# awentzonline/tartangan

Measured on AMD Instinct MI355X. Metric: images/sec (G+D step), higher is better.
Workload: dtype f32; 1 GPU; 128:3 SA-GAN cnn G+D step (R1 penalty, Adam x2, EMA), 128x128 RGB, batch 64/GPU, global batch 64; trainer=cnn, gan_config=128:3, global_batch=64, parallelism=dp1, hip_graphs=True

## Files before the change

tartangan_amd/csrc/conv.hip:

```cpp
#include <cstdlib>
#include <type_traits>
#include <utility>

#include "common.h"

namespace {

typedef float f32x16 __attribute__((ext_vector_type(16)));
typedef float f32x4 __attribute__((ext_vector_type(4)));

constexpr int CT_THREADS = 256;

template <int TH_, int TW_, int NI_>
struct Geo {
  static constexpr int TH = TH_, TW = TW_, NI = NI_, NPIX = TH_ * TW_ * NI_;
  static_assert(NPIX == 512 || NPIX == 256 || NPIX == 64, "a pixel tile is 512 / 256 pixels (waves split pixels) or 64 (waves split K)");
  static constexpr int PPW = (NPIX == 64) ? 64 : NPIX / 4;
  static_assert(TW_ % 4 == 0, "rows are staged as float4");
};
using G4 = Geo<4, 4, 16>;
using G8 = Geo<8, 8, 4>;
using G16 = Geo<16, 16, 1>;
using GX = Geo<8, 32, 1>;
using G4k = Geo<4, 4, 4>;
// ... 692 lines not shown
#pragma unroll
        for (int m = 0; m < MT; ++m)
          a[m] = DGRAD ? wl[lane_a + (g * KG) * F::RS + m * MF * 9 - tap] : wl[lane_a + m * MF * F::RS + (g * KG) * 9 + tap];
#pragma unroll
        for (int n = 0; n < NT; ++n) b[n] = pl[lane_b[n] + (g * KG) * P::CIS + kh * P::PWS + kw];
#pragma unroll
        for (int m = 0; m < MT; ++m)
#pragma unroll
          for (int n = 0; n < NT; ++n) {
            if constexpr (MF == 32)
              acc[m][n] = __builtin_amdgcn_mfma_f32_32x32x2f32(a[m], b[n], acc[m][n], 0, 0, 0);
            else
              acc[m][n] = __builtin_amdgcn_mfma_f32_16x16x4f32(a[m], b[n], acc[m][n], 0, 0, 0);
          }
      }
    }
    if (prio) __builtin_amdgcn_s_setprio(3);
    if (DB) buf ^= 1;
  }
#ifdef TG_DIAG_STAMPS
  {
    const uint64_t st_c1 = __builtin_amdgcn_s_memtime(), st_r1 = __builtin_amdgcn_s_memrealtime();
    const int slot = blockIdx.y * gridDim.x + blockIdx.x;
    if (threadIdx.x == 0 && slot < TG_DIAG_SLOTS) { tg_diag_stamps[2 * slot] = st_c1 - st_c0; tg_diag_stamps[2 * slot + 1] = st_r1 - st_r0; }
    st_mfma += st_c1 - st_last;
    if (lane == 0 && slot < TG_DIAG_SLOTS) {
      unsigned long long* ph = tg_diag_phases + (slot * 4 + wave) * 4;
      ph[0] = st_wait; ph[1] = st_bar; ph[2] = st_issue; ph[3] = st_mfma;
    }
  }
#endif
  if constexpr (WK) {
    __syncthreads();
    float* red = lds;
#pragma unroll
    for (int m = 0; m < MT; ++m)
#pragma unroll
      for (int n = 0; n < NT; ++n)
#pragma unroll
        for (int r = 0; r < NREG; ++r) red[(((wave * MT + m) * NT + n) * NREG + r) * 64 + lane] = acc[m][n][r];
    __syncthreads();
    constexpr int PW_ = MT * NT * NREG * 64;
#pragma unroll
    for (int m = 0; m < MT; ++m)
#pragma unroll
      for (int n = 0; n < NT; ++n)
#pragma unroll
        for (int r = 0; r < NREG; ++r) {
          const int e = ((m * NT + n) * NREG + r) * 64 + lane;
          acc[m][n][r] = (red[e] + red[PW_ + e]) + (red[2 * PW_ + e] + red[3 * PW_ + e]);
        }
  }
#ifdef TG_DIAG_STAMPS
  if ((xcd_swizzle & 2) && acc[0][0][0] != 12345.678f) return;
#endif
  Core::epilogue(acc, bias, residual, y, s, tc, co0, pix0, j, h, wave);
#ifdef TG_DIAG_STAMPS
  {
    const uint64_t e0 = __builtin_amdgcn_s_memtime();
    asm volatile("s_waitcnt vmcnt(0)" ::: "memory");
    const uint64_t e1 = __builtin_amdgcn_s_memtime();
    const int slot = blockIdx.y * gridDim.x + blockIdx.x;
    if (lane == 0 && slot < TG_DIAG_SLOTS) {
      unsigned long long* ph = tg_diag_life + (slot * 4 + wave) * 4;
      ph[0] = st_c0 - st_begin; ph[1] = e0 - st_c0; ph[2] = e1 - e0; ph[3] = st_setup - st_begin;
    }
  }
#endif
}

template <int CO, int PX>
__global__ void __launch_bounds__(256)
conv1x1_direct_kernel(const float* __restrict__ x, const float* __restrict__ w, const float* __restrict__ bias,
                      const float* __restrict__ residual, float* __restrict__ y, int Cin, int Cout, int HW, int w_so, int w_si) {
  __shared__ __attribute__((aligned(16))) float wl[1024];
  for (int e = threadIdx.x; e < Cin * CO; e += 256) {
    const int ci = e / CO, co = e - ci * CO;
    wl[e] = co < Cout ? w[co * w_so + ci * w_si] : 0.f;
  }
  __syncthreads();
  const int b = blockIdx.y;
  const int p = (blockIdx.x * 256 + threadIdx.x) * PX;
  if (p >= HW) return;
  const float* xb = x + (int64_t)b * Cin * HW + p;
  float acc[CO][PX];
#pragma unroll
  for (int co = 0; co < CO; ++co)
#pragma unroll
    for (int u = 0; u < PX; ++u) acc[co][u] = 0.f;
#pragma unroll 4
  for (int ci = 0; ci < Cin; ++ci) {
    float xv[PX];
    if (PX == 4) {
      const float4 t = *reinterpret_cast<const float4*>(xb + (int64_t)ci * HW);
      xv[0] = t.x; xv[1] = t.y; xv[2] = t.z; xv[3] = t.w;
    } else {
      xv[0] = xb[(int64_t)ci * HW];
    }
#pragma unroll
    for (int c4 = 0; c4 < CO / 4; ++c4) {
      const float4 wv = *reinterpret_cast<const float4*>(&wl[ci * CO + 4 * c4]);
      const float ww[4] = {wv.x, wv.y, wv.z, wv.w};
#pragma unroll
      for (int k = 0; k < 4; ++k)
#pragma unroll
        for (int u = 0; u < PX; ++u) acc[4 * c4 + k][u] = fmaf(ww[k], xv[u], acc[4 * c4 + k][u]);
    }
  }
  const int64_t ob = (int64_t)b * Cout * HW + p;
#pragma unroll
  for (int co = 0; co < CO; ++co) {
    if (co >= Cout) break;
    const float bv = bias ? bias[co] : 0.f;
    float o[PX];
#pragma unroll
    for (int u = 0; u < PX; ++u) o[u] = acc[co][u] + bv;
    const int64_t off = ob + (int64_t)co * HW;
    if (PX == 4) {
      if (residual) {
        const float4 r = *reinterpret_cast<const float4*>(residual + off);
        o[0] += r.x; o[1] += r.y; o[2] += r.z; o[3] += r.w;
      }
      *reinterpret_cast<float4*>(y + off) = make_float4(o[0], o[1], o[2], o[3]);
    } else {
      if (residual) o[0] += residual[off];
      y[off] = o[0];
    }
  }
}

template <int CO>
static int launch_conv1x1_direct(const float* x, const float* w, const float* bias, const float* residual, float* y, Shape s,
                                 bool dgrad, hipStream_t st) {
  const int HW = s.H * s.W;
  const int w_so = dgrad ? 1 : s.Cin, w_si = dgrad ? s.Cout : 1;
  const bool vec = (HW % 4 == 0) && tg_aligned16(x) && tg_aligned16(y) && (!residual || tg_aligned16(residual));
  if (vec) {
    dim3 grid((HW / 4 + 255) / 256, s.B);
    conv1x1_direct_kernel<CO, 4><<<grid, 256, 0, st>>>(x, w, bias, residual, y, s.Cin, s.Cout, HW, w_so, w_si);
  } else {
    dim3 grid((HW + 255) / 256, s.B);
    conv1x1_direct_kernel<CO, 1><<<grid, 256, 0, st>>>(x, w, bias, residual, y, s.Cin, s.Cout, HW, w_so, w_si);
  }
  return tg_launch_status();
}
static inline int conv1x1_co(int Cout) { return Cout <= 4 ? 4 : 8; }
static inline bool conv1x1_direct_ok(const Shape& s) { return s.Cout <= 8 && s.Cin * conv1x1_co(s.Cout) <= 1024 && s.B <= 65535; }
static int launch_conv1x1(const float* x, const float* w, const float* bias, const float* residual, float* y, Shape s, bool dgrad,
                          hipStream_t st) {
  if (s.Cout <= 4) return launch_conv1x1_direct<4>(x, w, bias, residual, y, s, dgrad, st);
  return launch_conv1x1_direct<8>(x, w, bias, residual, y, s, dgrad, st);
}

struct ChanSegs {
  float* p[3];
  int start[4];
  __device__ __forceinline__ int find(int c) const { return c >= start[2] ? 2 : (c >= start[1] ? 1 : 0); }
  __device__ __forceinline__ int width(int k) const { return start[k + 1] - start[k]; }
};
static inline ChanSegs one_seg(const float* p, int channels) {
  ChanSegs g;
  g.p[0] = g.p[1] = g.p[2] = const_cast<float*>(p);
  g.start[0] = 0; g.start[1] = g.start[2] = g.start[3] = channels;
  return g;
}
static inline ChanSegs three_segs(const float* p0, const float* p1, const float* p2, int c0, int c1, int c2) {
  ChanSegs g;
  g.p[0] = const_cast<float*>(p0); g.p[1] = const_cast<float*>(p1); g.p[2] = const_cast<float*>(p2);
  g.start[0] = 0; g.start[1] = c0; g.start[2] = c0 + c1; g.start[3] = c0 + c1 + c2;
  return g;
}

template <int NCO>
__global__ void __launch_bounds__(256)
conv1x1_mfma_kernel(ChanSegs xs, const float* __restrict__ w, const float* __restrict__ bias,
                    const float* __restrict__ residual, ChanSegs ys, int Cin, int Cout, int HW, int64_t quads,
                    int w_so, int w_si) {
  const int lane = threadIdx.x & 63, j = lane & 15, h = lane >> 4;
  const int64_t q = ((int64_t)blockIdx.x * 4 + (threadIdx.x >> 6)) * 16 + j;
  const bool live = q < quads;
  const int qpp = HW >> 2;
  const int64_t b = live ? q / qpp : 0;
  const int p = live ? (int)(q - b * qpp) * 4 : 0;
  f32x4 acc[NCO][4];
#pragma unroll
  for (int m = 0; m < NCO; ++m)
#pragma unroll
    for (int r = 0; r < 4; ++r) acc[m][r] = f32x4{0.f, 0.f, 0.f, 0.f};
  int wrow[NCO];
#pragma unroll
  for (int m = 0; m < NCO; ++m) wrow[m] = min(16 * m + j, Cout - 1) * w_so;
  constexpr int U = 4;
  for (int k0 = 0; k0 < Cin; k0 += 4 * U) {
    float4 xv[U];
    float a[U][NCO];
#pragma unroll
    for (int u = 0; u < U; ++u) {
      const int ci = k0 + 4 * u + h;
      const bool ok = live && ci < Cin;
      const int cc = min(ci, Cin - 1);
      const int k = xs.find(cc);
      const float* src = xs.p[k] + ((b * xs.width(k) + (cc - xs.start[k])) * HW + p);
      xv[u] = ok ? *reinterpret_cast<const float4*>(src) : make_float4(0.f, 0.f, 0.f, 0.f);
#pragma unroll
      for (int m = 0; m < NCO; ++m) a[u][m] = (ci < Cin) ? w[wrow[m] + cc * w_si] : 0.f;
    }
#pragma unroll
    for (int u = 0; u < U; ++u) {
      const float bx[4] = {xv[u].x, xv[u].y, xv[u].z, xv[u].w};
#pragma unroll
      for (int m = 0; m < NCO; ++m)
#pragma unroll
        for (int r = 0; r < 4; ++r) acc[m][r] = __builtin_amdgcn_mfma_f32_16x16x4f32(a[u][m], bx[r], acc[m][r], 0, 0, 0);
    }
  }
  if (!live) return;
  const float* rb = residual ? residual + (b * Cout) * HW + p : nullptr;
#pragma unroll
  for (int m = 0; m < NCO; ++m)
#pragma unroll
    for (int i = 0; i < 4; ++i) {
      const int co = 16 * m + 4 * h + i;
      if (co >= Cout) continue;
      const float bv = bias ? bias[co] : 0.f;
      float4 o = make_float4(acc[m][0][i] + bv, acc[m][1][i] + bv, acc[m][2][i] + bv, acc[m][3][i] + bv);
      if (rb) {
        const float4 t = *reinterpret_cast<const float4*>(rb + (int64_t)co * HW);
        o.x += t.x; o.y += t.y; o.z += t.z; o.w += t.w;
      }
      const int k = ys.find(co);
      *reinterpret_cast<float4*>(ys.p[k] + ((b * ys.width(k) + (co - ys.start[k])) * HW + p)) = o;
    }
}

static inline bool conv1x1_mfma_ok(const float* x, const float* residual, const float* y, const Shape& s) {
  return (s.H * s.W) % 4 == 0 && s.Cout <= 128 && tg_aligned16(x) && tg_aligned16(y) && (!residual || tg_aligned16(residual));
}
static int launch_conv1x1_segs(ChanSegs xs, const float* w, const float* bias, const float* residual, ChanSegs ys, Shape s, bool dgrad,
                               hipStream_t st) {
  const int HW = s.H * s.W;
  const int64_t quads = (int64_t)s.B * (HW / 4);
  const int w_so = dgrad ? 1 : s.Cin, w_si = dgrad ? s.Cout : 1;
  const unsigned grid = (unsigned)((quads + 63) / 64);
  const int nco = (s.Cout + 15) / 16;
#define TG_1X1(N) conv1x1_mfma_kernel<N><<<grid, 256, 0, st>>>(xs, w, bias, residual, ys, s.Cin, s.Cout, HW, quads, w_so, w_si)
  if (nco <= 1) TG_1X1(1);
  else if (nco == 2) TG_1X1(2);
  else if (nco <= 4) TG_1X1(4);
  else TG_1X1(8);
#undef TG_1X1
  return tg_launch_status();
}
static int launch_conv1x1_mfma(const float* x, const float* w, const float* bias, const float* residual, float* y, Shape s, bool dgrad,
                               hipStream_t st) {
  return launch_conv1x1_segs(one_seg(x, s.Cin), w, bias, residual, one_seg(y, s.Cout), s, dgrad, st);
}

template <int KS> struct WgCfg {
  static constexpr int CKW = (KS == 3) ? 16 : 32;
  static constexpr int KK = KS * KS;
  static constexpr int NCOL = CKW * KK;
  static constexpr int NT = (NCOL + 15) / 16;
};
constexpr int WG_GYS = 256 + 4;

template <class G, int CT>
struct GyStager {
  static constexpr int Q = G::TW / 4;
  static constexpr int ROWS_PER_CO = G::NI * G::TH;
  static constexpr int ROWS = CT * ROWS_PER_CO;
  static constexpr int NV = (ROWS * Q + CT_THREADS - 1) / CT_THREADS;
  float4 v[NV];

  __device__ __forceinline__ void load(const float* __restrict__ gy, const Shape& s, int co0, const TileCoord& tc, bool vec) {
#pragma unroll
    for (int i = 0; i < NV; ++i) {
      const int e = threadIdx.x + i * CT_THREADS;
      float4 val = make_float4(0.f, 0.f, 0.f, 0.f);
      if (e < ROWS * Q) {
        const int q = e % Q, row = e / Q;
        const int r = row % G::TH;
        const int t = row / G::TH;
        const int img = t % G::NI, co = t / G::NI;
        const int b = tc.b0 + img, hh = tc.h0 + r, ww = tc.w0 + 4 * q;
        if (b < s.B && co0 + co < s.Cout && hh < s.H && ww < s.W) {
          const float* base = gy + ((((int64_t)tc.b0 * s.Cout + co0) * s.H + tc.h0) * s.W + tc.w0);
          const float* src = base + (__umul24(__umul24(img, s.Cout) + co, s.H * s.W) + __umul24(r, s.W) + 4 * q);
          if (vec) {
            val = *reinterpret_cast<const float4*>(src);
          } else {
            val.x = src[0];
            if (ww + 1 < s.W) val.y = src[1];
            if (ww + 2 < s.W) val.z = src[2];
            if (ww + 3 < s.W) val.w = src[3];
          }
        }
      }
      v[i] = val;
    }
  }

  __device__ __forceinline__ void store(float* __restrict__ gl) const {
#pragma unroll
    for (int i = 0; i < NV; ++i) {
      const int e = threadIdx.x + i * CT_THREADS;
      if (e < ROWS * Q) {
        const int q = e % Q, row = e / Q;
        const int co = row / ROWS_PER_CO, prow = row % ROWS_PER_CO;
        *reinterpret_cast<float4*>(gl + co * WG_GYS + prow * G::TW + 4 * q) = v[i];
      }
    }
  }

  static_assert(ROWS_PER_CO * Q == 64, "one channel of a gy tile = one wave's worth of float4");
  __device__ __forceinline__ void add_channel_sums(float* acc ) const {
#pragma unroll
    for (int i = 0; i < NV; ++i) acc[i] += wave_sum((v[i].x + v[i].y) + (v[i].z + v[i].w));
  }
};

template <class G, int KS, int MTW>
__global__ void __launch_bounds__(CT_THREADS)
conv_wgrad_kernel(const float* __restrict__ x, const float* __restrict__ gy, float* __restrict__ part,
                  float* __restrict__ bias_part , Shape s, int ntiles, int S, int vec_x, int vec_gy) {
  using P = Patch<G, KS>;
  using C = WgCfg<KS>;
  constexpr int CKW = C::CKW, KK = C::KK, NT = C::NT, CT = 16 * MTW;
  constexpr int PATCH = CKW * P::CIS, GYT = CT * WG_GYS;
  constexpr int RED = 4 * MTW * NT * 4 * 64;
  constexpr int LDS_FLOATS = (PATCH + GYT) > RED ? (PATCH + GYT) : RED;
  __shared__ __attribute__((aligned(16))) float lds[LDS_FLOATS];
  float* pl = lds;
  float* gl = lds + PATCH;

  const int lane = threadIdx.x & 63, wave = threadIdx.x >> 6;
  const int j = lane & 15, h = lane >> 4;
  const int co0 = blockIdx.y * CT, ci0 = blockIdx.z * CKW;
  const int split = blockIdx.x;

  int colbase[NT];
#pragma unroll
  for (int n = 0; n < NT; ++n) {
    const int col = n * 16 + j;
    const int ci = col / KK, tap = col % KK;
    colbase[n] = (col < C::NCOL) ? (ci * P::CIS + (tap / KS) * P::PWS + (tap % KS)) : 0;
  }
  const int lane_b = pix_off<G, KS>(wave * 64) + h;
  const int lane_a = j * WG_GYS + wave * 64 + h;

  f32x4 acc[MTW][NT];
#pragma unroll
  for (int m = 0; m < MTW; ++m)
#pragma unroll
    for (int n = 0; n < NT; ++n) acc[m][n] = f32x4{0.f, 0.f, 0.f, 0.f};

  PatchStager<G, KS, CKW> ps;
  GyStager<G, CT> gs;
  const bool do_bias = (bias_part != nullptr) && (blockIdx.z == 0);
  float bsum[GyStager<G, CT>::NV];
#pragma unroll
  for (int i = 0; i < GyStager<G, CT>::NV; ++i) bsum[i] = 0.f;
  if (split < ntiles) {
    const TileCoord tc = decode_tile<G>(split, s.H, s.W);
    ps.load(x, s, s.Cin, ci0, tc, vec_x);
    gs.load(gy, s, co0, tc, vec_gy);
  }
  for (int t = split; t < ntiles; t += S) {
    __syncthreads();
    ps.store(pl);
    gs.store(gl);
    if (do_bias) gs.add_channel_sums(bsum);
    __syncthreads();
    if (t + S < ntiles) {
      const TileCoord tn = decode_tile<G>(t + S, s.H, s.W);
      ps.load(x, s, s.Cin, ci0, tn, vec_x);
      gs.load(gy, s, co0, tn, vec_gy);
    }
#pragma unroll
    for (int g = 0; g < 16; ++g) {
      constexpr int PPI = G::TH * G::TW;
      const int pg = 4 * g;
      const int goff = ((pg / PPI) * P::PH + (pg % PPI) / G::TW) * P::PWS + (pg % G::TW);
      float a[MTW], b[NT];
#pragma unroll
      for (int m = 0; m < MTW; ++m) a[m] = gl[lane_a + m * 16 * WG_GYS + 4 * g];
#pragma unroll
      for (int n = 0; n < NT; ++n) b[n] = pl[colbase[n] + lane_b + goff];
#pragma unroll
      for (int m = 0; m < MTW; ++m)
#pragma unroll
        for (int n = 0; n < NT; ++n) acc[m][n] = __builtin_amdgcn_mfma_f32_16x16x4f32(a[m], b[n], acc[m][n], 0, 0, 0);
    }
  }

  if (do_bias && lane == 0) {
#pragma unroll
    for (int i = 0; i < GyStager<G, CT>::NV; ++i) {
      const int co = co0 + 4 * i + wave;
      if (4 * i + wave < CT && co < s.Cout) bias_part[(int64_t)split * s.Cout + co] = bsum[i];
    }
  }
  __syncthreads();
// ... 25 lines not shown
                      float* __restrict__ bias_part , Shape s, int ntiles, int S) {
  static_assert(G::NPIX == 256 && WG_GYS == 4 * WGD_GYQ, "256-pixel tiles");
  using P = DPatch<G>;
  constexpr int KK = 9, CT = 16 * MTW, NCOL = CKW * KK, NT = (NCOL + 15) / 16;
  constexpr int PCH = CKW * P::CPC, GCH = CT * WGD_GYQ;
  constexpr int PCHP = dma_pad(PCH), GCHP = dma_pad(GCH);
  constexpr int NVP = (PCHP + CT_THREADS - 1) / CT_THREADS, NVG = (GCHP + CT_THREADS - 1) / CT_THREADS;
  constexpr int PBUF = PCHP * 4, BUF = PBUF + GCHP * 4;
  constexpr int RED = 4 * MTW * NT * 4 * 64 + 4 * CT;
  constexpr int LDSF = ((DB ? 2 : 1) * BUF > RED) ? (DB ? 2 : 1) * BUF : RED;
  __shared__ __attribute__((aligned(16))) float lds[LDSF];

  const int lane = threadIdx.x & 63, wave = wave_index();
  if (s.prio) __builtin_amdgcn_s_setprio(3);
  const int j = lane & 15, h = lane >> 4;
  const int co0 = blockIdx.y * CT, ci0 = blockIdx.z * CKW;
  const int split = blockIdx.x;
  const uint32_t HW = (uint32_t)(s.H * s.W);

  int colbase[NT];
#pragma unroll
  for (int n = 0; n < NT; ++n) {
    const int col = n * 16 + j;
    const int ci = col / KK, tap = col % KK;
    colbase[n] = (col < NCOL) ? (ci * P::CIS + (tap / 3) * P::PWS + (tap % 3)) : 0;
  }
  const int lane_b = P::pix(wave * 64) + h;
  const int lane_a = j * WG_GYS + wave * 64 + h;

  f32x4 acc[MTW][NT];
#pragma unroll
  for (int m = 0; m < MTW; ++m)
#pragma unroll
    for (int n = 0; n < NT; ++n) acc[m][n] = f32x4{0.f, 0.f, 0.f, 0.f};
  const bool do_bias = (bias_part != nullptr) && (blockIdx.z == 0);
  float bsum[MTW];
#pragma unroll
  for (int m = 0; m < MTW; ++m) bsum[m] = 0.f;

  const int cvalid = min(CKW, s.Cin - ci0);
  auto issue = [&](int t, float* buf) {
    const TileCoord tc = decode_tile<G>(t, s.H, s.W);
    const char* xb = reinterpret_cast<const char*>(x) + ((int64_t)tc.b0 * s.Cin + ci0) * HW * 4;
    const int64_t xbytes = ((int64_t)(s.B - tc.b0) * s.Cin - ci0) * HW * 4;
    const char* gb = reinterpret_cast<const char*>(gy) + ((int64_t)tc.b0 * s.Cout + co0) * HW * 4;
    const int64_t gbytes = ((int64_t)(s.B - tc.b0) * s.Cout - co0) * HW * 4;
    const __amdgpu_buffer_rsrc_t rx = __builtin_amdgcn_make_buffer_rsrc(const_cast<char*>(xb), 0, (int)xbytes, 0x00020000);
    const __amdgpu_buffer_rsrc_t rg = __builtin_amdgcn_make_buffer_rsrc(const_cast<char*>(gb), 0, (int)gbytes, 0x00020000);
#pragma unroll
    for (int i = 0; i < NVP; ++i) {
      const int e = i * CT_THREADS + threadIdx.x;
      const int ci = e / P::CPC, rem = e % P::CPC;
      const int row = rem / P::QR, q = rem % P::QR;
      const int img = row / P::PH, r = row % P::PH;
      const int hh = tc.h0 + r - 1, ww = tc.w0 - 4 + 4 * q;
      const bool ok = (rem < P::RAW / 4) && (ci < cvalid) && (tc.b0 + img < s.B) && (hh >= 0) && (hh < s.H) && (ww >= 0) && (ww < s.W);
      const uint32_t off = ok ? (__umul24(__umul24(img, s.Cin) + ci, HW) + __umul24(hh, s.W) + ww) << 2 : DMA_OOB;
      if ((i + 1) * CT_THREADS <= PCHP || i * CT_THREADS + wave * 64 < PCHP) dma16(rx, buf + (i * CT_THREADS + wave * 64) * 4, off);
    }
#pragma unroll
    for (int i = 0; i < NVG; ++i) {
      const int e = i * CT_THREADS + threadIdx.x;
      const int co = e / WGD_GYQ, q = e % WGD_GYQ;
      const int p = 4 * q;
      const int img = p / (G::TH * G::TW), rem = p % (G::TH * G::TW);
      const int hh = tc.h0 + rem / G::TW, ww = tc.w0 + rem % G::TW;
      const bool ok = (e < GCH) && (q < 64) && (co0 + co < s.Cout) && (tc.b0 + img < s.B) && (hh < s.H) && (ww < s.W);
      const uint32_t off = ok ? (__umul24(__umul24(img, s.Cout) + co, HW) + __umul24(hh, s.W) + ww) << 2 : DMA_OOB;
      if ((i + 1) * CT_THREADS <= GCHP || i * CT_THREADS + wave * 64 < GCHP) dma16(rg, buf + PBUF + (i * CT_THREADS + wave * 64) * 4, off);
    }
  };
  auto compute = [&](const float* buf) {
    const float* pl = buf;
    const float* gl = buf + PBUF;
    if (s.prio) __builtin_amdgcn_s_setprio(0);
#pragma unroll
    for (int g = 0; g < 16; ++g) {
      constexpr int PPI = G::TH * G::TW;
      const int pg = 4 * g;
      const int goff = ((pg / PPI) * P::PH + (pg % PPI) / G::TW) * P::PWS + (pg % G::TW);
      float a[MTW], b[NT];
#pragma unroll
      for (int m = 0; m < MTW; ++m) a[m] = gl[lane_a + m * 16 * WG_GYS + 4 * g];
#pragma unroll
      for (int n = 0; n < NT; ++n) b[n] = pl[colbase[n] + lane_b + goff];
#pragma unroll
      for (int m = 0; m < MTW; ++m) bsum[m] += a[m];
#pragma unroll
      for (int m = 0; m < MTW; ++m)
#pragma unroll
        for (int n = 0; n < NT; ++n) acc[m][n] = __builtin_amdgcn_mfma_f32_16x16x4f32(a[m], b[n], acc[m][n], 0, 0, 0);
    }
    if (s.prio) __builtin_amdgcn_s_setprio(3);
  };

  if constexpr (DB) {
    if (split < ntiles) issue(split, lds);
    int buf = 0;
    for (int t = split; t < ntiles; t += S) {
      asm volatile("s_waitcnt vmcnt(0)" ::: "memory");
      __syncthreads();
      if (t + S < ntiles) issue(t + S, lds + (buf ^ 1) * BUF);
      compute(lds + buf * BUF);
      buf ^= 1;
    }
  } else {
    for (int t = split; t < ntiles; t += S) {
      __syncthreads();
      issue(t, lds);
      asm volatile("s_waitcnt vmcnt(0)" ::: "memory");
      __syncthreads();
      compute(lds);
    }
  }

  __syncthreads();
  float* red = lds;
#pragma unroll
  for (int m = 0; m < MTW; ++m)
#pragma unroll
    for (int n = 0; n < NT; ++n)
#pragma unroll
      for (int r = 0; r < 4; ++r) red[(((wave * MTW + m) * NT + n) * 4 + r) * 64 + lane] = acc[m][n][r];
  constexpr int PER_WAVE = MTW * NT * 4 * 64;
  float* bred = lds + 4 * PER_WAVE;
  if (do_bias) {
#pragma unroll
    for (int m = 0; m < MTW; ++m) {
      float v = bsum[m];
      v += __shfl_xor(v, 16, 64);
      v += __shfl_xor(v, 32, 64);
      if (h == 0) bred[wave * CT + m * 16 + j] = v;
    }
  }
  __syncthreads();
  for (int e = threadIdx.x; e < PER_WAVE; e += CT_THREADS) {
    const float v = (red[e] + red[PER_WAVE + e]) + (red[2 * PER_WAVE + e] + red[3 * PER_WAVE + e]);
    const int l = e & 63, q = e >> 6;
    const int r = q & 3, n = (q >> 2) % NT, m = (q >> 2) / NT;
    const int col = n * 16 + (l & 15);
    const int co = co0 + m * 16 + (l >> 4) * 4 + r;
    const int ci = ci0 + col / KK, tap = col % KK;
    if (col < NCOL && co < s.Cout && ci < s.Cin)
      part[(((int64_t)split * s.Cout + co) * s.Cin + ci) * KK + tap] = v;
  }
  if (do_bias && threadIdx.x < CT && co0 + (int)threadIdx.x < s.Cout) {
    const int c = threadIdx.x;
    bias_part[(int64_t)split * s.Cout + co0 + c] = (bred[c] + bred[CT + c]) + (bred[2 * CT + c] + bred[3 * CT + c]);
  }
}

template <int MT, int NT>
__global__ void __launch_bounds__(256)
conv1x1_wgrad_stream_kernel(const float* __restrict__ x, ChanSegs gys, float* __restrict__ part,
                            float* __restrict__ bias_part , int Cin, int Cout, int HW, int64_t groups, int S) {
  __shared__ float red[4 * MT * NT * 4 * 64 + 4 * 16 * MT];
  const int lane = threadIdx.x & 63, wave = threadIdx.x >> 6, j = lane & 15, h = lane >> 4;
  const int co0 = blockIdx.y * 16 * MT, ci0 = blockIdx.z * 16 * NT, split = blockIdx.x;
  const int64_t g_begin = groups * split / S, g_end = groups * (split + 1) / S;
  const int64_t n = g_end - g_begin;
  const int64_t w_begin = g_begin + n * wave / 4, w_end = g_begin + n * (wave + 1) / 4;
  const int gpp = HW >> 4;
  int64_t arow[MT], brow[NT], aimg[MT];
  const float* abase[MT];
#pragma unroll
  for (int m = 0; m < MT; ++m) {
    const int co = min(co0 + 16 * m + j, Cout - 1), k = gys.find(co);
    abase[m] = gys.p[k];
    aimg[m] = (int64_t)gys.width(k) * HW;
    arow[m] = (int64_t)(co - gys.start[k]) * HW + 4 * h;
  }
#pragma unroll
  for (int t = 0; t < NT; ++t) brow[t] = (int64_t)min(ci0 + 16 * t + j, Cin - 1) * HW + 4 * h;
  f32x4 acc[MT][NT];
#pragma unroll
  for (int m = 0; m < MT; ++m)
#pragma unroll
    for (int t = 0; t < NT; ++t) acc[m][t] = f32x4{0.f, 0.f, 0.f, 0.f};
  float bsum[MT];
#pragma unroll
  for (int m = 0; m < MT; ++m) bsum[m] = 0.f;
  constexpr int U = 4;
  for (int64_t g0 = w_begin; g0 < w_end; g0 += U) {
    float4 ga[U][MT], xb[U][NT];
#pragma unroll
    for (int u = 0; u < U; ++u) {
      const int64_t g = g0 + u;
      const bool ok = g < w_end;
      const int64_t b = ok ? g / gpp : 0;
      const int64_t p = ok ? (g - b * gpp) * 16 : 0;
#pragma unroll
      for (int m = 0; m < MT; ++m)
        ga[u][m] = ok ? *reinterpret_cast<const float4*>(abase[m] + b * aimg[m] + arow[m] + p) : make_float4(0.f, 0.f, 0.f, 0.f);
#pragma unroll
      for (int t = 0; t < NT; ++t)
        xb[u][t] = ok ? *reinterpret_cast<const float4*>(x + b * Cin * HW + brow[t] + p) : make_float4(0.f, 0.f, 0.f, 0.f);
    }
#pragma unroll
    for (int u = 0; u < U; ++u) {
#pragma unroll
      for (int m = 0; m < MT; ++m) bsum[m] += (ga[u][m].x + ga[u][m].y) + (ga[u][m].z + ga[u][m].w);
#pragma unroll
      for (int m = 0; m < MT; ++m) {
        const float av[4] = {ga[u][m].x, ga[u][m].y, ga[u][m].z, ga[u][m].w};
#pragma unroll
        for (int t = 0; t < NT; ++t) {
          const float bv[4] = {xb[u][t].x, xb[u][t].y, xb[u][t].z, xb[u][t].w};
#pragma unroll
          for (int r = 0; r < 4; ++r) acc[m][t] = __builtin_amdgcn_mfma_f32_16x16x4f32(av[r], bv[r], acc[m][t], 0, 0, 0);
        }
      }
    }
  }
  constexpr int PER_WAVE = MT * NT * 4 * 64;
#pragma unroll
  for (int m = 0; m < MT; ++m)
#pragma unroll
    for (int t = 0; t < NT; ++t)
#pragma unroll
      for (int i = 0; i < 4; ++i) red[wave * PER_WAVE + ((m * NT + t) * 4 + i) * 64 + lane] = acc[m][t][i];
  float* bred = red + 4 * PER_WAVE;
  const bool do_bias = bias_part != nullptr && blockIdx.z == 0;
  if (do_bias) {
#pragma unroll
    for (int m = 0; m < MT; ++m) {
      float v = bsum[m];
      v += __shfl_xor(v, 16, 64);
      v += __shfl_xor(v, 32, 64);
      if (h == 0) bred[wave * 16 * MT + 16 * m + j] = v;
    }
  }
  __syncthreads();
  for (int e = threadIdx.x; e < PER_WAVE; e += 256) {
    const float v = (red[e] + red[PER_WAVE + e]) + (red[2 * PER_WAVE + e] + red[3 * PER_WAVE + e]);
    const int l = e & 63, q = e >> 6;
    const int i = q & 3, t = (q >> 2) % NT, m = (q >> 2) / NT;
    const int co = co0 + 16 * m + 4 * (l >> 4) + i, ci = ci0 + 16 * t + (l & 15);
    if (co < Cout && ci < Cin) part[((int64_t)split * Cout + co) * Cin + ci] = v;
  }
  if (do_bias && threadIdx.x < 16 * MT && co0 + (int)threadIdx.x < Cout) {
    const int c = threadIdx.x;
    bias_part[(int64_t)split * Cout + co0 + c] = (bred[c] + bred[16 * MT + c]) + (bred[2 * 16 * MT + c] + bred[3 * 16 * MT + c]);
  }
}

static int conv1x1_mode();
static inline bool conv1x1_wgrad_stream_ok(const float* x, const float* gy, const Shape& s) {
  return conv1x1_mode() != 0 && (s.H * s.W) % 16 == 0 && tg_aligned16(x) && tg_aligned16(gy);
}
static int launch_conv1x1_wgrad_segs(const float* x, ChanSegs gy, float* part, float* bias_part, Shape s, int S, hipStream_t st) {
  const int HW = s.H * s.W;
  const int64_t groups = (int64_t)s.B * (HW / 16);
  const int mt = s.Cout > 16 ? 2 : 1, nt = s.Cin > 16 ? 2 : 1;
  dim3 grid(S, (s.Cout + 16 * mt - 1) / (16 * mt), (s.Cin + 16 * nt - 1) / (16 * nt));
  if (mt == 1 && nt == 1) conv1x1_wgrad_stream_kernel<1, 1><<<grid, 256, 0, st>>>(x, gy, part, bias_part, s.Cin, s.Cout, HW, groups, S);
  else if (mt == 1) conv1x1_wgrad_stream_kernel<1, 2><<<grid, 256, 0, st>>>(x, gy, part, bias_part, s.Cin, s.Cout, HW, groups, S);
  else if (nt == 1) conv1x1_wgrad_stream_kernel<2, 1><<<grid, 256, 0, st>>>(x, gy, part, bias_part, s.Cin, s.Cout, HW, groups, S);
  else conv1x1_wgrad_stream_kernel<2, 2><<<grid, 256, 0, st>>>(x, gy, part, bias_part, s.Cin, s.Cout, HW, groups, S);
  return tg_launch_status();
}
static int launch_conv1x1_wgrad_stream(const float* x, const float* gy, float* part, float* bias_part, Shape s, int S, hipStream_t st) {
  return launch_conv1x1_wgrad_segs(x, one_seg(gy, s.Cout), part, bias_part, s, S, st);
}

__device__ __forceinline__ void wgrad_reduce_block(int blk, const float* __restrict__ part, float* __restrict__ gw, int64_t E, int S,
                                                   const float* __restrict__ bias_part, float* __restrict__ gbias, int Cout,
                                                   int accumulate) {
  __shared__ float red[4][64];
  const int lane = threadIdx.x & 63, wave = threadIdx.x >> 6;
  const int eblocks = (int)((E + 63) / 64);
  const float* src = part;
  float* dst = gw;
  int64_t n = E, e = blk * 64ll + lane;
  if (blk >= eblocks) {
    src = bias_part; dst = gbias; n = Cout;
    e = (blk - eblocks) * 64ll + lane;
  }
  float a0 = 0.f, a1 = 0.f, a2 = 0.f, a3 = 0.f;
  if (e < n) {
    int sidx = wave;
    for (; sidx + 12 < S; sidx += 16) {
      a0 += src[(int64_t)sidx * n + e];
      a1 += src[(int64_t)(sidx + 4) * n + e];
      a2 += src[(int64_t)(sidx + 8) * n + e];
      a3 += src[(int64_t)(sidx + 12) * n + e];
    }
    for (; sidx < S; sidx += 4) a0 += src[(int64_t)sidx * n + e];
  }
  red[wave][lane] = (a0 + a1) + (a2 + a3);
  __syncthreads();
  if (wave == 0 && e < n) {
    const float r = (red[0][lane] + red[1][lane]) + (red[2][lane] + red[3][lane]);
    dst[e] = accumulate ? dst[e] + r : r;
  }
}

__global__ void __launch_bounds__(256) wgrad_reduce_kernel(const float* __restrict__ part, float* __restrict__ gw, int64_t E, int S,
                                                           const float* __restrict__ bias_part, float* __restrict__ gbias, int Cout,
                                                           int accumulate) {
  wgrad_reduce_block(blockIdx.x, part, gw, E, S, bias_part, gbias, Cout, accumulate);
}

constexpr int RB_MAX_ITEMS = 40;
struct ReduceItem {
  const float* part; float* gw; float* gbias;
  int64_t E;
  int S, Cout, accumulate, pad;
};
struct ReduceBatch {
  int n;
  int block_end[RB_MAX_ITEMS];
  ReduceItem item[RB_MAX_ITEMS];
};
__global__ void __launch_bounds__(256) wgrad_reduce_batch_kernel(ReduceBatch rb) {
  int i = 0;
  while (i + 1 < rb.n && (int)blockIdx.x >= rb.block_end[i]) ++i;
  const ReduceItem it = rb.item[i];
  const int blk = blockIdx.x - (i > 0 ? rb.block_end[i - 1] : 0);
  wgrad_reduce_block(blk, it.part, it.gw, it.E, it.S, it.gbias ? it.part + (int64_t)it.S * it.E : nullptr, it.gbias, it.Cout,
                     it.accumulate);
}

__global__ void __launch_bounds__(256) upconv_weights_kernel(const float* __restrict__ w, float* __restrict__ wp, int n ) {
  const int e = blockIdx.x * 256 + threadIdx.x;
  if (e >= n) return;
  float k[3][3];
#pragma unroll
  for (int i = 0; i < 9; ++i) k[i / 3][i % 3] = w[(int64_t)e * 9 + i];
#pragma unroll
  for (int dy = 0; dy < 2; ++dy)
#pragma unroll
    for (int dx = 0; dx < 2; ++dx) {
      float r[2][3];
#pragma unroll
      for (int c = 0; c < 3; ++c) {
        r[0][c] = dy == 0 ? k[0][c] : k[0][c] + k[1][c];
        r[1][c] = dy == 0 ? k[1][c] + k[2][c] : k[2][c];
      }
      float* o = wp + ((int64_t)(dy * 2 + dx) * n + e) * 4;
#pragma unroll
      for (int ty = 0; ty < 2; ++ty) {
        o[ty * 2 + 0] = dx == 0 ? r[ty][0] : r[ty][0] + r[ty][1];
        o[ty * 2 + 1] = dx == 0 ? r[ty][1] + r[ty][2] : r[ty][2];
      }
    }
}

template <class G, bool WK>
__global__ void __launch_bounds__(CT_THREADS)
conv_upfwd_kernel(const float* __restrict__ x, const float* __restrict__ wp, const float* __restrict__ bias,
                  const float* __restrict__ residual, float* __restrict__ y, Shape s, int vec_x, int vec_w) {
  constexpr int KS = 2, CT = 16, NT = 4, KG = 4;
  using P = Patch<G, KS>;
  using WT = WTile<KS, CT, WK>;
  constexpr int KK = WT::KK, CK = WT::CK, CTS = WT::CTS, NG = CK / KG, GSTEP = WK ? 4 : 1;
  static_assert(G::NPIX == (WK ? 64 : 256) && KK == 4 && NG % GSTEP == 0, "256-pixel tiles (or 64, K split over the waves), 2x2 windows");
  constexpr int STAGE = CK * P::CIS + 4 * WT::SIZE, REDF = WK ? 4 * 2 * NT * 4 * 64 : 0;
  __shared__ __attribute__((aligned(16))) float lds[STAGE > REDF ? STAGE : REDF];
  float* pl = lds;
  float* wl = lds + CK * P::CIS;
  const int lane = threadIdx.x & 63, wave = threadIdx.x >> 6;
  const int j = lane & 15, h = lane >> 4;
  const TileCoord tc = decode_tile<G>(blockIdx.x, s.H, s.W);
  const int co0 = blockIdx.y * CT;
// ... 1857 lines not shown
```

Baseline: 6982 images/s.

## Software-pipeline 1x1 conv MFMA kernels and split output channels across grid

Rewrites the 1x1 conv forward MFMA kernel so input and weight loads for upcoming K rounds are issued before the current round's MFMAs run, with R-deep register buffering. Output-channel blocks move onto a second grid dimension, processed one or two 16-channel blocks at a time, so waves carry fewer accumulators and the grid grows. Segment pointers become scalar registers and the single-segment case is specialised to skip the lookup. The wgrad stream kernel gets the same D-deep prefetch with an incremental batch/pixel index in place of per-group division. This trades more registers, and in the forward kernel re-reading the input once per channel block, for better latency hiding and occupancy.

```diff
diff --git a/tartangan_amd/csrc/conv.hip b/tartangan_amd/csrc/conv.hip
--- a/tartangan_amd/csrc/conv.hip
+++ b/tartangan_amd/csrc/conv.hip
@@ -868,11 +868,26 @@
   return launch_conv1x1_direct<8>(x, w, bias, residual, y, s, dgrad, st);
 }
 
+struct SegRegs {
+  float* base;
+  int64_t d1, d2;
+  int s1, s2, s3;
+  __device__ __forceinline__ int find(int c) const { return c >= s2 ? 2 : (c >= s1 ? 1 : 0); }
+  __device__ __forceinline__ int64_t delta(int k) const { return k == 2 ? d2 : (k == 1 ? d1 : (int64_t)0); }
+  __device__ __forceinline__ int first(int k) const { return k == 2 ? s2 : (k == 1 ? s1 : 0); }
+  __device__ __forceinline__ int width(int k) const { return k == 2 ? s3 - s2 : (k == 1 ? s2 - s1 : s1); }
+};
 struct ChanSegs {
   float* p[3];
   int start[4];
-  __device__ __forceinline__ int find(int c) const { return c >= start[2] ? 2 : (c >= start[1] ? 1 : 0); }
-  __device__ __forceinline__ int width(int k) const { return start[k + 1] - start[k]; }
+  __device__ __forceinline__ SegRegs regs() const {
+    SegRegs r;
+    r.base = p[0];
+    r.d1 = p[1] - p[0]; r.d2 = p[2] - p[0];
+    r.s1 = start[1]; r.s2 = start[2]; r.s3 = start[3];
+    asm volatile("" : "+s"(r.d1), "+s"(r.d2), "+s"(r.s1), "+s"(r.s2), "+s"(r.s3));
+    return r;
+  }
 };
 static inline ChanSegs one_seg(const float* p, int channels) {
   ChanSegs g;
@@ -887,83 +902,108 @@
   return g;
 }
 
-template <int NCO>
+template <int NB, int R, bool SEGS>
 __global__ void __launch_bounds__(256)
-conv1x1_mfma_kernel(ChanSegs xs, const float* __restrict__ w, const float* __restrict__ bias,
-                    const float* __restrict__ residual, ChanSegs ys, int Cin, int Cout, int HW, int64_t quads,
+conv1x1_mfma_kernel(ChanSegs xs_arg, const float* __restrict__ w, const float* __restrict__ bias,
+                    const float* __restrict__ residual, ChanSegs ys_arg, int Cin, int Cout, int HW, int64_t quads,
                     int w_so, int w_si) {
+  const SegRegs xs = xs_arg.regs(), ys = ys_arg.regs();
   const int lane = threadIdx.x & 63, j = lane & 15, h = lane >> 4;
-  const int64_t q = ((int64_t)blockIdx.x * 4 + (threadIdx.x >> 6)) * 16 + j;
+  const int wave = __builtin_amdgcn_readfirstlane(threadIdx.x >> 6);
+  const int64_t q = ((int64_t)blockIdx.x * 4 + wave) * 16 + j;
   const bool live = q < quads;
   const int qpp = HW >> 2;
-  const int64_t b = live ? q / qpp : 0;
+  const int64_t b = !live ? 0 : (quads <= 0x7fffffff ? (int64_t)((uint32_t)q / (uint32_t)qpp) : q / qpp);
   const int p = live ? (int)(q - b * qpp) * 4 : 0;
-  f32x4 acc[NCO][4];
-#pragma unroll
-  for (int m = 0; m < NCO; ++m)
+  const int mb = blockIdx.y * NB;
+  f32x4 acc[NB][4];
+#pragma unroll
+  for (int m = 0; m < NB; ++m)
 #pragma unroll
     for (int r = 0; r < 4; ++r) acc[m][r] = f32x4{0.f, 0.f, 0.f, 0.f};
-  int wrow[NCO];
-#pragma unroll
-  for (int m = 0; m < NCO; ++m) wrow[m] = min(16 * m + j, Cout - 1) * w_so;
+  int wrow[NB];
+#pragma unroll
+  for (int m = 0; m < NB; ++m) wrow[m] = min(16 * (mb + m) + j, Cout - 1) * w_so;
   constexpr int U = 4;
-  for (int k0 = 0; k0 < Cin; k0 += 4 * U) {
-    float4 xv[U];
-    float a[U][NCO];
+  float4 xv[R][U];
+  float a[R][U][NB];
+  auto load_round = [&](float4 (&xr)[U], float (&ar)[U][NB], int k0) {
 #pragma unroll
     for (int u = 0; u < U; ++u) {
       const int ci = k0 + 4 * u + h;
       const bool ok = live && ci < Cin;
       const int cc = min(ci, Cin - 1);
-      const int k = xs.find(cc);
-      const float* src = xs.p[k] + ((b * xs.width(k) + (cc - xs.start[k])) * HW + p);
-      xv[u] = ok ? *reinterpret_cast<const float4*>(src) : make_float4(0.f, 0.f, 0.f, 0.f);
-#pragma unroll
-      for (int m = 0; m < NCO; ++m) a[u][m] = (ci < Cin) ? w[wrow[m] + cc * w_si] : 0.f;
-    }
-#pragma unroll
-    for (int u = 0; u < U; ++u) {
-      const float bx[4] = {xv[u].x, xv[u].y, xv[u].z, xv[u].w};
-#pragma unroll
-      for (int m = 0; m < NCO; ++m)
-#pragma unroll
-        for (int r = 0; r < 4; ++r) acc[m][r] = __builtin_amdgcn_mfma_f32_16x16x4f32(a[u][m], bx[r], acc[m][r], 0, 0, 0);
+      const int k = SEGS ? xs.find(cc) : 0;
+      const float* src = xs.base + (xs.delta(k) + (b * xs.width(k) + (cc - xs.first(k))) * HW + p);
+      xr[u] = ok ? *reinterpret_cast<const float4*>(src) : make_float4(0.f, 0.f, 0.f, 0.f);
+#pragma unroll
+      for (int m = 0; m < NB; ++m) ar[u][m] = (ci < Cin) ? w[wrow[m] + cc * w_si] : 0.f;
+    }
+  };
+#pragma unroll
+  for (int r = 0; r < R; ++r)
+    if (16 * r < Cin) load_round(xv[r], a[r], 16 * r);
+  float bv[NB][4];
+  float4 res[NB][4];
+  const float* rb = (residual && live) ? residual + (b * Cout) * HW + p : nullptr;
+#pragma unroll
+  for (int m = 0; m < NB; ++m)
+#pragma unroll
+    for (int i = 0; i < 4; ++i) {
+      const int co = 16 * (mb + m) + 4 * h + i;
+      bv[m][i] = (bias && co < Cout) ? bias[co] : 0.f;
+      res[m][i] = (rb && co < Cout) ? *reinterpret_cast<const float4*>(rb + (int64_t)co * HW) : make_float4(0.f, 0.f, 0.f, 0.f);
+    }
+  for (int k0 = 0; k0 < Cin; k0 += 16 * R) {
+#pragma unroll
+    for (int r = 0; r < R; ++r) {
+      if (k0 + 16 * r >= Cin) break;
+#pragma unroll
+      for (int u = 0; u < U; ++u) {
+        const float bx[4] = {xv[r][u].x, xv[r][u].y, xv[r][u].z, xv[r][u].w};
+#pragma unroll
+        for (int m = 0; m < NB; ++m)
+#pragma unroll
+          for (int t = 0; t < 4; ++t) acc[m][t] = __builtin_amdgcn_mfma_f32_16x16x4f32(a[r][u][m], bx[t], acc[m][t], 0, 0, 0);
+      }
+      if (k0 + 16 * (r + R) < Cin) load_round(xv[r], a[r], k0 + 16 * (r + R));
     }
   }
   if (!live) return;
-  const float* rb = residual ? residual + (b * Cout) * HW + p : nullptr;
-#pragma unroll
-  for (int m = 0; m < NCO; ++m)
+#pragma unroll
+  for (int m = 0; m < NB; ++m)
 #pragma unroll
     for (int i = 0; i < 4; ++i) {
-      const int co = 16 * m + 4 * h + i;
+      const int co = 16 * (mb + m) + 4 * h + i;
       if (co >= Cout) continue;
-      const float bv = bias ? bias[co] : 0.f;
-      float4 o = make_float4(acc[m][0][i] + bv, acc[m][1][i] + bv, acc[m][2][i] + bv, acc[m][3][i] + bv);
-      if (rb) {
-        const float4 t = *reinterpret_cast<const float4*>(rb + (int64_t)co * HW);
-        o.x += t.x; o.y += t.y; o.z += t.z; o.w += t.w;
-      }
-      const int k = ys.find(co);
-      *reinterpret_cast<float4*>(ys.p[k] + ((b * ys.width(k) + (co - ys.start[k])) * HW + p)) = o;
+      float4 o = make_float4(acc[m][0][i] + bv[m][i], acc[m][1][i] + bv[m][i], acc[m][2][i] + bv[m][i], acc[m][3][i] + bv[m][i]);
+      if (rb) { o.x += res[m][i].x; o.y += res[m][i].y; o.z += res[m][i].z; o.w += res[m][i].w; }
+      const int k = SEGS ? ys.find(co) : 0;
+      *reinterpret_cast<float4*>(ys.base + (ys.delta(k) + (b * ys.width(k) + (co - ys.first(k))) * HW + p)) = o;
     }
 }
 
 static inline bool conv1x1_mfma_ok(const float* x, const float* residual, const float* y, const Shape& s) {
   return (s.H * s.W) % 4 == 0 && s.Cout <= 128 && tg_aligned16(x) && tg_aligned16(y) && (!residual || tg_aligned16(residual));
 }
+static constexpr int64_t CONV1X1_NB2_WAVES = 2048;
 static int launch_conv1x1_segs(ChanSegs xs, const float* w, const float* bias, const float* residual, ChanSegs ys, Shape s, bool dgrad,
                                hipStream_t st) {
   const int HW = s.H * s.W;
   const int64_t quads = (int64_t)s.B * (HW / 4);
   const int w_so = dgrad ? 1 : s.Cin, w_si = dgrad ? s.Cout : 1;
-  const unsigned grid = (unsigned)((quads + 63) / 64);
+  const int64_t wgs = (quads + 63) / 64;
   const int nco = (s.Cout + 15) / 16;
-#define TG_1X1(N) conv1x1_mfma_kernel<N><<<grid, 256, 0, st>>>(xs, w, bias, residual, ys, s.Cin, s.Cout, HW, quads, w_so, w_si)
-  if (nco <= 1) TG_1X1(1);
-  else if (nco == 2) TG_1X1(2);
-  else if (nco <= 4) TG_1X1(4);
-  else TG_1X1(8);
+  const bool two = nco >= 2 && 4 * wgs * ((nco + 1) / 2) >= CONV1X1_NB2_WAVES;
+  const dim3 grid((unsigned)wgs, two ? (nco + 1) / 2 : nco);
+  const bool segs = xs.start[1] != xs.start[3] || ys.start[1] != ys.start[3];
+#define TG_1X1(NB, R)                                                                                                              \
+  do {                                                                                                                             \
+    if (segs) conv1x1_mfma_kernel<NB, R, true><<<grid, 256, 0, st>>>(xs, w, bias, residual, ys, s.Cin, s.Cout, HW, quads, w_so, w_si); \
+    else conv1x1_mfma_kernel<NB, R, false><<<grid, 256, 0, st>>>(xs, w, bias, residual, ys, s.Cin, s.Cout, HW, quads, w_so, w_si);     \
+  } while (0)
+  if (s.Cin <= 32) { if (two) TG_1X1(2, 2); else TG_1X1(1, 2); }
+  else { if (two) TG_1X1(2, 4); else TG_1X1(1, 4); }
 #undef TG_1X1
   return tg_launch_status();
 }
@@ -1295,10 +1335,12 @@
 
 template <int MT, int NT>
 __global__ void __launch_bounds__(256)
-conv1x1_wgrad_stream_kernel(const float* __restrict__ x, ChanSegs gys, float* __restrict__ part,
+conv1x1_wgrad_stream_kernel(const float* __restrict__ x, ChanSegs gys_arg, float* __restrict__ part,
                             float* __restrict__ bias_part , int Cin, int Cout, int HW, int64_t groups, int S) {
+  const SegRegs gys = gys_arg.regs();
   __shared__ float red[4 * MT * NT * 4 * 64 + 4 * 16 * MT];
-  const int lane = threadIdx.x & 63, wave = threadIdx.x >> 6, j = lane & 15, h = lane >> 4;
+  const int lane = threadIdx.x & 63, j = lane & 15, h = lane >> 4;
+  const int wave = __builtin_amdgcn_readfirstlane(threadIdx.x >> 6);
   const int co0 = blockIdx.y * 16 * MT, ci0 = blockIdx.z * 16 * NT, split = blockIdx.x;
   const int64_t g_begin = groups * split / S, g_end = groups * (split + 1) / S;
   const int64_t n = g_end - g_begin;
@@ -1309,9 +1351,9 @@
 #pragma unroll
   for (int m = 0; m < MT; ++m) {
     const int co = min(co0 + 16 * m + j, Cout - 1), k = gys.find(co);
-    abase[m] = gys.p[k];
+    abase[m] = gys.base + gys.delta(k);
     aimg[m] = (int64_t)gys.width(k) * HW;
-    arow[m] = (int64_t)(co - gys.start[k]) * HW + 4 * h;
+    arow[m] = (int64_t)(co - gys.first(k)) * HW + 4 * h;
   }
 #pragma unroll
   for (int t = 0; t < NT; ++t) brow[t] = (int64_t)min(ci0 + 16 * t + j, Cin - 1) * HW + 4 * h;
@@ -1323,24 +1365,33 @@
   float bsum[MT];
 #pragma unroll
   for (int m = 0; m < MT; ++m) bsum[m] = 0.f;
-  constexpr int U = 4;
-  for (int64_t g0 = w_begin; g0 < w_end; g0 += U) {
-    float4 ga[U][MT], xb[U][NT];
-#pragma unroll
-    for (int u = 0; u < U; ++u) {
-      const int64_t g = g0 + u;
-      const bool ok = g < w_end;
-      const int64_t b = ok ? g / gpp : 0;
-      const int64_t p = ok ? (g - b * gpp) * 16 : 0;
-#pragma unroll
-      for (int m = 0; m < MT; ++m)
-        ga[u][m] = ok ? *reinterpret_cast<const float4*>(abase[m] + b * aimg[m] + arow[m] + p) : make_float4(0.f, 0.f, 0.f, 0.f);
-#pragma unroll
-      for (int t = 0; t < NT; ++t)
-        xb[u][t] = ok ? *reinterpret_cast<const float4*>(x + b * Cin * HW + brow[t] + p) : make_float4(0.f, 0.f, 0.f, 0.f);
-    }
-#pragma unroll
-    for (int u = 0; u < U; ++u) {
+  constexpr int D = (MT + NT == 4) ? 5 : 8;
+  const int64_t w_end4 = w_begin + ((w_end - w_begin + 3) & ~(int64_t)3);
+  int64_t lg = w_begin;
+  int64_t lb = lg / gpp;
+  int lp = (int)(lg - lb * gpp) * 16;
+  float4 ga[D][MT], xb[D][NT];
+  auto load_group = [&](float4 (&gc)[MT], float4 (&xc)[NT]) {
+    const bool ok = lg < w_end;
+    const int64_t b = ok ? lb : 0;
+    const int64_t p = ok ? lp : 0;
+#pragma unroll
+    for (int m = 0; m < MT; ++m)
+      gc[m] = ok ? *reinterpret_cast<const float4*>(abase[m] + b * aimg[m] + arow[m] + p) : make_float4(0.f, 0.f, 0.f, 0.f);
+#pragma unroll
+    for (int t = 0; t < NT; ++t)
+      xc[t] = ok ? *reinterpret_cast<const float4*>(x + b * Cin * HW + brow[t] + p) : make_float4(0.f, 0.f, 0.f, 0.f);
+    ++lg;
+    lp += 16;
+    if (lp == HW) { lp = 0; ++lb; }
+  };
+#pragma unroll
+  for (int u = 0; u < D; ++u)
+    if (w_begin + u < w_end4) load_group(ga[u], xb[u]);
+  for (int64_t g0 = w_begin; g0 < w_end4; g0 += D) {
+#pragma unroll
+    for (int u = 0; u < D; ++u) {
+      if (g0 + u >= w_end4) break;
 #pragma unroll
       for (int m = 0; m < MT; ++m) bsum[m] += (ga[u][m].x + ga[u][m].y) + (ga[u][m].z + ga[u][m].w);
 #pragma unroll
@@ -1353,6 +1404,7 @@
           for (int r = 0; r < 4; ++r) acc[m][t] = __builtin_amdgcn_mfma_f32_16x16x4f32(av[r], bv[r], acc[m][t], 0, 0, 0);
         }
       }
+      if (g0 + u + D < w_end4) load_group(ga[u], xb[u]);
     }
   }
   constexpr int PER_WAVE = MT * NT * 4 * 64;
```

After: 7061 images/s (median of 6 runs). 1.01x the previous value.
